# cemlyn007/ale-libtorch-ppo

Measured on AMD Instinct MI355X. Metric: env steps/sec (whole node), Breakout 84x84x4, higher is better.
Workload: dtype bf16; 1 GPU; Breakout-shaped synthetic, 128 envs/GPU x T=128, A=4, H=512, 4 epochs x 4 minibatches of 4096 (configs[1], v0.yaml update shape); envs_per_gpu=128, horizon=128, epochs=4, minibatches=4, parallelism=dp1, frames=raw u8 [E,2,210,160] pairs resident in HBM, rollout_planes=fp32, update_graph=False, dp_schedule_forced=False

## Files before the change

ale-libtorch-ppo_amd/csrc/api_core.hip:

```cpp
#include "api_internal.hpp"

using namespace aleppo;

namespace aleppo {

static thread_local std::string g_err;
int set_err(Ctx *c, int code, const std::string &msg) {
  if (c)
    c->err = msg;
  g_err = msg;
  return code;
}

static thread_local const Tuning *g_tuning = nullptr;
Tuning tuning_from_env() {
  auto flag = [](const char *name, bool dflt) {
    const char *e = std::getenv(name);
    return e ? std::atoi(e) != 0 : dflt;
  };
  Tuning t;
  t.patch_conv = !flag("ALEPPO_GENERIC_CONV", false);
  t.fc_pipe = flag("ALEPPO_FC_PIPE", true);
  t.fused_fwd = flag("ALEPPO_FWD_FUSED", true);
  if (const char *e = std::getenv("ALEPPO_BWD_FUSED"))
// ... 313 lines not shown
  CK(dalloc(&c->mask_counts, 4096 * 4, c->stream));
  CK(dalloc(&c->P, PT * 4, c->stream));
  CK(dalloc(&c->G, PT * 4, c->stream));
  CK(dalloc(&c->M1, PT * 4, c->stream));
  CK(dalloc(&c->M2, PT * 4, c->stream));
  if (c->prec == ALEPPO_BF16)
    CK(dalloc(reinterpret_cast<char **>(&c->Pc), PT * 2, c->stream));
  else
    c->Pc = c->P;
  CK(dalloc(reinterpret_cast<char **>(&c->W2d), (size_t)4 * 32 * 256 * ts, c->stream));
  CK(dalloc(reinterpret_cast<char **>(&c->W3d), (size_t)64 * 576 * ts, c->stream));
  CK(dalloc(reinterpret_cast<char **>(&c->WfcT), (size_t)FC_IN * H * ts, c->stream));
  const size_t mb = (size_t)c->maxB;
  CK(dalloc(reinterpret_cast<char **>(&c->a1), mb * A1_PIX * A1_C * ts, c->stream));
  CK(dalloc(reinterpret_cast<char **>(&c->a2), mb * A2_PIX * A2_C * ts, c->stream));
  CK(dalloc(reinterpret_cast<char **>(&c->a3), mb * FC_IN * ts, c->stream));
  CK(dalloc(reinterpret_cast<char **>(&c->dz1), mb * A1_PIX * A1_C * ts, c->stream));
  CK(dalloc(reinterpret_cast<char **>(&c->dz2), mb * A2_PIX * A2_C * ts, c->stream));
  CK(dalloc(reinterpret_cast<char **>(&c->dz3), mb * FC_IN * ts, c->stream));
  CK(dalloc(&c->h, (size_t)FC_FWD_MAX_PARTS * mb * H * 4, c->stream));
  CK(dalloc(&c->hpart, (size_t)FC_SPLITS * E * H * 4, c->stream));
  CK(dalloc(reinterpret_cast<char **>(&c->dh), mb * H * ts, c->stream));
  CK(dalloc(&c->logits_b, mb * A * 4, c->stream));
  CK(dalloc(&c->values_b, mb * 4, c->stream));
  c->slab_off[0] = 0;
  const size_t sl[10] = {(size_t)MAXS_C1 * 32 * 256,       (size_t)MAXS_C1 * 32, (size_t)MAXS_C2 * 64 * 512,
                         (size_t)MAXS_C2 * 64,              (size_t)MAXS_C3 * 64 * 576, (size_t)MAXS_C3 * 64,
                         (size_t)MAXS_FC * H * FC_IN,       (size_t)MAXS_HEAD * H, (size_t)MAXS_HEAD * (A + 1) * H,
                         (size_t)MAXS_HEAD * (A + 1)};
  for (int i = 0; i < 10; ++i)
    c->slab_off[i + 1] = c->slab_off[i] + align64(sl[i]);
  c->slab_floats = c->slab_off[10];
  CK(dalloc(&c->slab, c->slab_floats * 4, c->stream));
  CK(dalloc(&c->sumsq_part, 1024 * 4, c->stream));
  CK(dalloc(&c->adv_stats, 64, c->stream));
  CK(dalloc(&c->hyper_blk, HYPER_BLOCK * 4, c->stream));
  CK(hipHostMalloc(reinterpret_cast<void **>(&c->h_hyper_blk), HYPER_BLOCK * 4, hipHostMallocDefault));
  CK(hipStreamSynchronize(c->stream));
#undef CK
  *out = c;
  return ALEPPO_OK;
}

extern "C" void aleppo_destroy(aleppo_ctx *c) {
  if (!c)
    return;
  set_tuning(nullptr);
  (void)hipSetDevice(c->cfg.device_ordinal);
  if (c->h_go)
    __atomic_store_n(c->h_go, ~0ull, __ATOMIC_RELEASE);
  for (hipStream_t st : {c->wg_stream, c->comm_stream, c->stream})
    if (st)
      hipStreamSynchronize(st);
  if (c->graph_exec)
    hipGraphExecDestroy(c->graph_exec);
  if (c->graph)
    hipGraphDestroy(c->graph);
  if (c->nccl_comm)
    ncclCommDestroy(static_cast<ncclComm_t>(c->nccl_comm));
  void *dev[] = {c->obs,   c->step_rec, c->values_tm, c->logits_tm, c->actions_tm, c->lut,     c->d_start,
                 c->d_frames, c->d_noise, c->d_err,  c->d_done, c->adv_n,     c->ret_n,      c->oldlp_n, c->act_n,
                 c->mask_n, c->mask_counts, c->P,    c->G,         c->M1,      c->M2,
                 c->W2d,   c->W3d,      c->WfcT,      c->a1,        c->a2,         c->a3,      c->dz1,
                 c->dz2,   c->dz3,      c->h,         c->hpart,     c->dh,        c->logits_b,   c->values_b, c->slab,
                 c->sumsq_part, c->metric_ps, c->metric_red, c->grad_norms, c->adv_stats, c->stage_u8, c->stage_obs,
                 c->adam_sched, c->rb_tmp[0], c->rb_tmp[1], c->order, c->act_p, c->oldlp_p, c->adv_p,
                 c->ret_p,  c->mask_p,   c->mask_counts_ep, c->shuf_keys, c->val_n, c->val_p, c->advn_part,
// ... 319 lines not shown
```

ale-libtorch-ppo_amd/csrc/api_train.hip:

```cpp
#include "api_internal.hpp"

using namespace aleppo;

int aleppo::ensure_metric_storage(aleppo_ctx *c, int epochs, int M, long B) {
  const size_t need = (size_t)epochs * M * B;
  if (need > c->metric_cap) {
    retire(c, c->metric_ps);
    c->metric_ps = nullptr;
    HIPCHK(c, dalloc(&c->metric_ps, need * 7 * 4, c->stream));
    c->metric_cap = need;
  }
  const size_t nm = (size_t)epochs * M;
  if (nm > c->metric_red_cap) {
    retire(c, c->metric_red);
    retire(c, c->grad_norms);
    retire(c, c->adam_sched);
    retire(c, c->advn_part);
    retire(c, c->advn_stats);
    retire_host(c, c->h_metric_red);
    retire_host(c, c->h_adam_sched);
    retire_host(c, c->h_advn_stats);
    c->metric_red = c->grad_norms = c->h_metric_red = c->adam_sched = c->h_adam_sched = nullptr;
    c->advn_part = nullptr;
    c->advn_stats = c->h_advn_stats = nullptr;
// ... 50 lines not shown
    HIPCHK(c, hipHostMalloc(reinterpret_cast<void **>(&c->h_kl_beta), 16, hipHostMallocDefault));
  }
  if (c->kl_cap < c->metric_cap) {
    retire(c, c->kl_ps);
    c->kl_ps = nullptr;
    c->kl_cap = 0;
    c->last_kl = false;
    HIPCHK(c, dalloc(&c->kl_ps, c->metric_cap * 4, c->stream));
    c->kl_cap = c->metric_cap;
  }
  return ALEPPO_OK;
}

int aleppo::ensure_val_storage(aleppo_ctx *c) {
  if (!c->val_n)
    HIPCHK(c, dalloc(&c->val_n, (size_t)c->N * c->rsz, c->stream));
  return ALEPPO_OK;
}

static uint64_t splitmix64(uint64_t x) {
  uint64_t z = x + 0x9E3779B97F4A7C15ull;
  z = (z ^ (z >> 30)) * 0xBF58476D1CE4E5B9ull;
  z = (z ^ (z >> 27)) * 0x94D049BB133111EBull;
  return z ^ (z >> 31);
}
static int feistel_half_width(long N) {
  int w = 0;
  while ((1L << w) < N)
    ++w;
  w = std::max(w, 2);
  return (w + 1) / 2;
}

static bool fuse_tail_env() {
  static const bool v = [] {
    const char *e = getenv("ALEPPO_FUSE_TAIL_REDUCE");
    return !e || atoi(e) != 0;
  }();
  return v;
}
static bool bwd_streams_env() {
  static const bool v = [] {
    const char *e = std::getenv("ALEPPO_BWD_STREAMS");
    return !(e && std::atoi(e) == 1);
  }();
  return v;
}

static inline size_t record_index(bool per_epoch, size_t period, size_t i) { return per_epoch ? i : i % period; }

struct Planes {
  const int *act;
  void *oldlp, *adv, *ret, *vold;
  const uint8_t *mask;
  const int32_t *order;
  float *counts;
  int ncounts;
  size_t epoch_stride;
  long B;
  int M;
  size_t offset(int ep, int mb) const { return (size_t)ep * epoch_stride + (size_t)mb * B; }
  size_t record(int ep, int mb) const { return record_index(order != nullptr, (size_t)M, (size_t)ep * M + mb); }
  const int32_t *idx(int ep) const { return order ? order + (size_t)ep * epoch_stride : nullptr; }
};

struct UpdatePlan {
  int epochs, M, nm;
  long N, B;
  bool shuffle, vclip, val_transpose, advn, klpen, dp, two, bwd_fused, fuse_tail;
  hipStream_t s, sw;
  ncclComm_t comm;
  Hyper hp;
  const float *hpd;
  int shuf_h, nblk_head, nblk_sq;
  size_t fs;
  float *sW1, *sB1, *sW2, *sB2, *sW3, *sB3, *sWfc, *sBfc, *sWh, *sBh;
  Planes pl;
};

static int plan_update(aleppo_ctx *c, int epochs, int M, UpdatePlan *plan) {
  UpdatePlan &p = *plan;
  if (epochs <= 0 || M <= 0)
    return set_err(c, ALEPPO_ERR_INVALID_ARGUMENT, "epochs and num_mini_batches must be positive");
  const long N = c->batch_n;
  if (N <= 0)
    return set_err(c, ALEPPO_ERR_RUNTIME, "no batch: call aleppo_finish_rollout or aleppo_set_batch first");
  c->pre_acted = -1;
  if (N % M != 0)
    return set_err(c, ALEPPO_ERR_RUNTIME, "Batch size must be divisible by num_mini_batches");
  const long B = N / M;
  if (B > c->maxB)
    return set_err(c, ALEPPO_ERR_INVALID_ARGUMENT, "minibatch larger than config.max_minibatch");
  if (M > 4096)
    return set_err(c, ALEPPO_ERR_INVALID_ARGUMENT, "num_mini_batches > 4096");
  if (c->world > 1 && !c->nccl_comm)
    return set_err(c, ALEPPO_ERR_RUNTIME, "world_size > 1 but aleppo_comm_init was not called");
  p.epochs = epochs;
  p.M = M;
  p.nm = epochs * M;
  p.N = N;
  p.B = B;
  p.vclip = c->value_clip;
  if (p.vclip && c->val_src == Ctx::VAL_NONE)
    return set_err(c, ALEPPO_ERR_RUNTIME,
                   "ALEPPO_OPT_VALUE_CLIP needs the batch's old values: call aleppo_set_batch_values after aleppo_set_batch");
  int rc = ensure_metric_storage(c, epochs, M, B);
  if (rc)
    return rc;
  p.shuffle = c->shuffle;
  p.advn = c->adv_norm_mb;
  p.klpen = c->kl_pen;
  if (p.klpen && (rc = ensure_kl_storage(c)))
    return rc;
  if (p.shuffle && (rc = ensure_shuffle_storage(c, epochs, N)))
    return rc;
  if (p.vclip && (rc = ensure_val_storage(c)))
    return rc;
  p.val_transpose = p.vclip && c->val_src == Ctx::VAL_ROLLOUT;
  p.comm = static_cast<ncclComm_t>(c->nccl_comm);
  p.dp = c->world > 1 || (c->nccl_comm && c->force_comm);
  if (!c->wg_stream)
    HIPCHK(c, hipStreamCreateWithFlags(&c->wg_stream, hipStreamNonBlocking));
  if (p.dp && !c->comm_stream)
    HIPCHK(c, hipStreamCreateWithFlags(&c->comm_stream, hipStreamNonBlocking));
  p.s = c->stream;
  p.hp = c->hyper;
  p.hpd = c->hyper_blk;
  p.shuf_h = feistel_half_width(N);

  p.sW1 = c->slab + c->slab_off[0], p.sB1 = c->slab + c->slab_off[1], p.sW2 = c->slab + c->slab_off[2];
  p.sB2 = c->slab + c->slab_off[3], p.sW3 = c->slab + c->slab_off[4], p.sB3 = c->slab + c->slab_off[5];
  p.sWfc = c->slab + c->slab_off[6], p.sBfc = c->slab + c->slab_off[7], p.sWh = c->slab + c->slab_off[8];
  p.sBh = c->slab + c->slab_off[9];
  p.fs = c->metric_cap;
  p.nblk_head = (int)std::min<long>(MAXS_HEAD, (B + 15) / 16);
  p.nblk_sq = (int)std::min<size_t>(800, (c->L.off[P_W1] + 4095) / 4096);

  p.two = bwd_streams_env() && !c->serial_update;
  p.bwd_fused = (c->tune.fused_bwd == 2 || (c->tune.fused_bwd == 1 && B >= 2048)) && c->prec == ALEPPO_BF16 &&
                use_patch_kernels() && !p.dp;
  p.sw = p.two ? c->wg_stream : p.s;
  p.fuse_tail = fuse_tail_env();

  Planes &pl = p.pl;
  pl.B = B;
  pl.M = M;
  if (p.shuffle) {
    pl.act = c->act_p, pl.oldlp = c->oldlp_p, pl.adv = c->adv_p, pl.ret = c->ret_p, pl.vold = c->val_p;
    pl.mask = c->mask_p, pl.order = c->order, pl.counts = c->mask_counts_ep;
    pl.ncounts = p.nm;
    pl.epoch_stride = (size_t)N;
  } else {
    pl.act = c->act_n, pl.oldlp = c->oldlp_n, pl.adv = c->adv_n, pl.ret = c->ret_n, pl.vold = c->val_n;
    pl.mask = c->mask_n, pl.order = nullptr, pl.counts = c->mask_counts;
    pl.ncounts = M;
    pl.epoch_stride = 0;
  }
  if (!p.vclip)
    pl.vold = nullptr;
  return ALEPPO_OK;
}

static int upload_call_scalars(aleppo_ctx *c, const UpdatePlan &p, double lr) {
  hipStream_t s = p.s;
  for (int i = 0; i < p.nm; ++i) {
    const double b1 = c->cfg.adam_beta1, b2 = c->cfg.adam_beta2, t = (double)(c->adam_step + i + 1);
    c->h_adam_sched[2 * i] = (float)(lr / (1.0 - std::pow(b1, t)));
    c->h_adam_sched[2 * i + 1] = (float)std::sqrt(1.0 - std::pow(b2, t));
  }
  HIPCHK(c, hipMemcpyAsync(c->adam_sched, c->h_adam_sched, (size_t)p.nm * 8, hipMemcpyHostToDevice, s));
  float *b = c->h_hyper_blk;
  std::memset(b, 0, HYPER_BLOCK * 4);
  b[HYPER_CLIP] = p.hp.clip;
  b[HYPER_VCLIP] = c->vclip_range_set ? c->value_clip_range : p.hp.clip;
  b[HYPER_CV] = p.hp.c_v;
// ... 52 lines not shown
  const size_t p0 = pl.offset(ep, mb), fs = p.fs;
  float *const mps = c->metric_ps + (size_t)mi * p.B;
  HeadTrainArgs ha{};
  ha.h = c->h;
  ha.Wh = Pf(c, P_WH);
  ha.bh = Pf(c, P_BH);
  ha.act = pl.act + p0;
  ha.oldlp = rp(c, pl.oldlp, p0 * A);
  ha.adv = rp(c, pl.adv, p0);
  ha.ret = rp(c, pl.ret, p0);
  ha.vold = pl.vold ? rp(c, pl.vold, p0) : nullptr;
  ha.mask = pl.mask + p0;
  ha.mask_count = pl.counts + pl.record(ep, mb);
  ha.dh = c->dh;
  ha.prec = c->prec;
  ha.ps_total = mps + 0 * fs, ha.ps_clipped = mps + 1 * fs, ha.ps_value = mps + 2 * fs, ha.ps_entropy = mps + 3 * fs;
  ha.ps_ratio = mps + 4 * fs, ha.ps_kl = mps + 5 * fs, ha.ps_cf = mps + 6 * fs;
  ha.slab_w = p.sWh;
  ha.slab_b = p.sBh;
  ha.nblk = p.nblk_head;
  ha.B = p.B;
  ha.H = c->H;
  ha.A = A;
  ha.hparts = hparts;
  ha.rt16 = c->rt16;
  ha.advs = p.advn ? c->advn_stats + pl.record(ep, mb) * 4 : nullptr;
  ha.klb = p.klpen ? c->kl_beta : nullptr;
  ha.ps_kle = p.klpen ? c->kl_ps + (size_t)mi * p.B : nullptr;
  launch_head_train(p.s, ha, p.hpd);
  prof_end(c, ALEPPO_K_HEAD);
}

struct SegList {
  ReduceSeg seg[10];
  int n = 0;
  void add(const ReduceSeg &r) { seg[n++] = r; }
  void add(const SegList &o) {
    for (int i = 0; i < o.n; ++i)
      seg[n++] = o.seg[i];
  }
};
static void reduce_beside(aleppo_ctx *c, const UpdatePlan &p, SegList &segs) {
  if (!p.two)
    return;
  prof_begin(c, ALEPPO_K_REDUCE, p.sw);
  launch_reduce_slabs(p.sw, segs.seg, segs.n, c->G);
  prof_end(c, ALEPPO_K_REDUCE, p.sw);
  segs.n = 0;
}

static int enqueue_conv_bwd_fused(aleppo_ctx *c, const UpdatePlan &p, const SampleMap &map, int S3,
                                  const SegList &late0, SegList &segs, int *S1) {
  const ParamLayout &L = c->L;
  segs.add(ReduceSeg{p.sW3, S3, 64 * 576, (long)L.off[P_W3]});
  segs.add(ReduceSeg{p.sB3, S3, 64, (long)L.off[P_B3]});
  segs.add(late0);
  reduce_beside(c, p, segs);
  prof_begin(c, ALEPPO_K_CONV_BWD);
  const int S2 = *S1 = patch_conv_bwd_fused(p.s, c->dz2, c->a1, c->obs, map, c->W2d, p.sW2, p.sB2, p.sW1, p.sB1, p.B);
  prof_end(c, ALEPPO_K_CONV_BWD);
  segs.add(ReduceSeg{p.sW2, S2, 64 * 512, (long)L.off[P_W2]});
  segs.add(ReduceSeg{p.sB2, S2, 64, (long)L.off[P_B2]});
  return ALEPPO_OK;
}
static int enqueue_conv_bwd_split(aleppo_ctx *c, const UpdatePlan &p, const SampleMap &map, int S3,
                                  const SegList &late0, SegList &segs, int *S1) {
  const ParamLayout &L = c->L;
  const int prec = c->prec;
  HIPCHK(c, fork_wgrad_stream(p, c->ev_dz2));
  prof_begin(c, ALEPPO_K_CONV2_DGRAD);
  conv2_dgrad(p.s, prec, c->dz2, c->W2d, c->a1, c->dz1, p.B);
  prof_end(c, ALEPPO_K_CONV2_DGRAD);
  prof_begin(c, ALEPPO_K_CONV2_WGRAD, p.sw);
  const int S2 = conv2_wgrad(p.sw, prec, c->dz2, c->a1, p.sW2, p.sB2, p.B);
  prof_end(c, ALEPPO_K_CONV2_WGRAD, p.sw);
  segs.add(ReduceSeg{p.sW3, S3, 64 * 576, (long)L.off[P_W3]});
  segs.add(ReduceSeg{p.sB3, S3, 64, (long)L.off[P_B3]});
  segs.add(ReduceSeg{p.sW2, S2, 64 * 512, (long)L.off[P_W2]});
  segs.add(ReduceSeg{p.sB2, S2, 64, (long)L.off[P_B2]});
  segs.add(late0);
  reduce_beside(c, p, segs);
  prof_begin(c, ALEPPO_K_CONV1_WGRAD);
  *S1 = conv1_wgrad(p.s, prec, c->dz1, c->obs, map, p.sW1, p.sB1, p.B);
  prof_end(c, ALEPPO_K_CONV1_WGRAD);
  return ALEPPO_OK;
}

static int enqueue_minibatch(aleppo_ctx *c, const UpdatePlan &p, int ep, int mb) {
  const int H = c->H, A = c->A, prec = c->prec, mi = ep * p.M + mb;
  const ParamLayout &L = c->L;
  const long B = p.B;
  hipStream_t s = p.s, sw = p.sw;
  SampleMap map = train_map(c, (long)mb * B);
  map.idx = p.pl.idx(ep);
  const int hparts = net_forward(c, c->obs, map, B, FC_FWD_MAX_PARTS);
  enqueue_head(c, p, ep, mb, hparts);
  HIPCHK(c, fork_wgrad_stream(p, c->ev_head));
  prof_begin(c, ALEPPO_K_FC_DGRAD);
  fc_dgrad(s, prec, c->dh, c->WfcT, c->a3, c->dz3, B, H);
  prof_end(c, ALEPPO_K_FC_DGRAD);
  prof_begin(c, ALEPPO_K_FC_WGRAD, sw);
  const bool fc_direct = fc_wgrad_slices(prec, B) == 1;
  const int Sfc = fc_wgrad(sw, prec, c->dh, c->a3, fc_direct ? c->G + L.off[P_WFC] : p.sWfc,
                           fc_direct ? c->G + L.off[P_BFC] : p.sBfc, B, H);
  prof_end(c, ALEPPO_K_FC_WGRAD, sw);
  SegList segs0;
  segs0.add(ReduceSeg{p.sWh, p.nblk_head, (long)(A + 1) * H, (long)L.off[P_WH]});
  segs0.add(ReduceSeg{p.sBh, p.nblk_head, (long)A + 1, (long)L.off[P_BH]});
  if (!fc_direct) {
    segs0.add(ReduceSeg{p.sWfc, Sfc, (long)H * FC_IN, (long)L.off[P_WFC]});
    segs0.add(ReduceSeg{p.sBfc, Sfc, (long)H, (long)L.off[P_BFC]});
  }
  if (p.dp) {
    HIPCHK(c, hipEventRecord(c->ev_bucket0, sw));
    HIPCHK(c, hipStreamWaitEvent(c->comm_stream, c->ev_bucket0, 0));
    prof_begin(c, ALEPPO_K_REDUCE, c->comm_stream);
    launch_reduce_slabs(c->comm_stream, segs0.seg, segs0.n, c->G);
    prof_end(c, ALEPPO_K_REDUCE, c->comm_stream);
    NCCLCHK(c, ncclAllReduce(c->G, c->G, L.bucket0_end, ncclFloat, ncclSum, p.comm, c->comm_stream));
    HIPCHK(c, hipEventRecord(c->ev_comm0, c->comm_stream));
    segs0.n = 0;
  }
  HIPCHK(c, fork_wgrad_stream(p, c->ev_dz3));
  prof_begin(c, ALEPPO_K_CONV3_DGRAD);
  conv3_dgrad(s, prec, c->dz3, c->W3d, c->a2, c->dz2, B);
  prof_end(c, ALEPPO_K_CONV3_DGRAD);
  prof_begin(c, ALEPPO_K_CONV3_WGRAD, sw);
  const int S3 = conv3_wgrad(sw, prec, c->dz3, c->a2, p.sW3, p.sB3, B);
  prof_end(c, ALEPPO_K_CONV3_WGRAD, sw);
  int S1 = 0;
  SegList segs;
  if (int rc = p.bwd_fused ? enqueue_conv_bwd_fused(c, p, map, S3, segs0, segs, &S1)
                           : enqueue_conv_bwd_split(c, p, map, S3, segs0, segs, &S1))
    return rc;
  if (p.two) {
    HIPCHK(c, hipEventRecord(c->ev_wg, sw));
    HIPCHK(c, hipStreamWaitEvent(s, c->ev_wg, 0));
  }
  ReduceSeg tail[2] = {{p.sW1, S1, 32 * 256, (long)L.off[P_W1]}, {p.sB1, S1, 32, (long)L.off[P_B1]}};
  if (p.dp || !p.fuse_tail) {
    segs.add(tail[0]);
    segs.add(tail[1]);
    tail[0].slab = tail[1].slab = nullptr;
  }
  if (segs.n) {
    prof_begin(c, ALEPPO_K_REDUCE);
    launch_reduce_slabs(s, segs.seg, segs.n, c->G);
    prof_end(c, ALEPPO_K_REDUCE);
  }
  if (p.dp) {
    HIPCHK(c, hipStreamWaitEvent(s, c->ev_comm0, 0));
    NCCLCHK(c, ncclAllReduce(c->G + L.bucket0_end, c->G + L.bucket0_end, L.total() - L.bucket0_end, ncclFloat, ncclSum,
                             p.comm, s));
  }
  prof_begin(c, ALEPPO_K_ADAM);
  const int nblk_norm = launch_sumsq(s, c->G, (long)L.off[P_W1], c->sumsq_part, p.nblk_sq, tail);
  launch_adam(s, c->P, c->G, nullptr, c->M1, c->M2, c->prec == ALEPPO_BF16 ? c->Pc : nullptr, c->WfcT, c->W3d, c->W2d, L,
              prec, c->sumsq_part, nblk_norm, p.hpd, c->adam_sched + 2 * mi, c->cfg.adam_beta1, c->cfg.adam_beta2,
              c->cfg.adam_eps, c->grad_norms + mi);
  prof_end(c, ALEPPO_K_ADAM);
  return ALEPPO_OK;
}

static int enqueue_epilogue(aleppo_ctx *c, const UpdatePlan &p) {
  const Planes &pl = p.pl;
  launch_metrics_reduce(p.s, c->metric_ps, p.fs, pl.mask, p.B, pl.ncounts, p.nm / pl.ncounts, c->metric_red,
                        p.klpen ? c->kl_ps : nullptr);
  if (p.dp)
    NCCLCHK(c, ncclAllReduce(c->metric_red, c->metric_red, (size_t)p.nm * METRIC_REC, ncclFloat, ncclSum, p.comm, p.s));
  return ALEPPO_OK;
}

static int enqueue_update(aleppo_ctx *c, const UpdatePlan &p) {
  if (int rc = enqueue_prologue(c, p))
    return rc;
  for (int ep = 0; ep < p.epochs; ++ep)
    for (int mb = 0; mb < p.M; ++mb)
      if (int rc = enqueue_minibatch(c, p, ep, mb))
        return rc;
  return enqueue_epilogue(c, p);
}

static Ctx::GraphKey graph_key(const UpdatePlan &p, const aleppo_ctx *c) {
  Ctx::GraphKey key;
  key.epochs = p.epochs;
  key.M = p.M;
  key.two = p.two ? 1 : 0;
  key.N = p.N;
  key.metric_ps = c->metric_ps;
// ... 169 lines not shown
```

ale-libtorch-ppo_amd/csrc/common.hpp:

```cpp
#pragma once
#include "../../include/aleppo.h"
#include <hip/hip_runtime.h>
#include <stdint.h>
#include <string>
#include <vector>

namespace aleppo {

constexpr int FRAME_PIX = 84 * 84;
constexpr int RAW_H = 210, RAW_W = 160;
constexpr int A1_PIX = 400, A1_C = 32;
constexpr int A2_PIX = 81, A2_C = 64;
constexpr int A3_PIX = 49, A3_C = 64;
constexpr int FC_IN = 3136;
constexpr int MAX_ACTIONS = 18;
constexpr int FC_SPLITS = 7;
constexpr int MAXS_C1 = 256, MAXS_C2 = 256, MAXS_C3 = 256, MAXS_FC = 8, MAXS_HEAD = 256;
constexpr int METRIC_REC = 9;

enum ParamId { P_WH = 0, P_BH, P_WFC, P_BFC, P_W3, P_B3, P_W2, P_B2, P_W1, P_B1, P_COUNT };
struct ParamLayout {
  size_t off[P_COUNT + 1];
  size_t size[P_COUNT];
  size_t bucket0_end;
// ... 263 lines not shown
void launch_bstat_reduce(hipStream_t s, const double *part, int nblk, double *sums, double *result);
void launch_bstat_finalise(hipStream_t s, const double *sums, double *result);
void launch_shuffle_gather(hipStream_t s, const uint32_t *rk, int h, long N, int epochs, int A, int32_t *order,
                           const int *act_n, const void *oldlp_n, const void *adv_n, const void *ret_n,
                           const void *val_n, const uint8_t *mask_n, int *act_p, void *oldlp_p, void *adv_p,
                           void *ret_p, void *val_p, uint8_t *mask_p, bool rt16);
struct HeadTrainArgs {
  const float *h, *Wh, *bh;
  const int *act;
  const void *oldlp, *adv, *ret, *vold;
  const uint8_t *mask;
  const float *mask_count;
  void *dh;
  int prec;
  float *ps_total, *ps_clipped, *ps_value, *ps_entropy, *ps_ratio, *ps_kl, *ps_cf;
  float *slab_w, *slab_b;
  int nblk;
  long B;
  int H, A;
  float *logits_out = nullptr, *values_out = nullptr;
  int hparts = 1;
  bool rt16 = false;
  const float *advs = nullptr, *klb = nullptr;
  float *ps_kle = nullptr;
};
void launch_head_train(hipStream_t s, const HeadTrainArgs &a, const float *hp);
struct ReduceSeg {
  const float *slab;
  int S;
  long n;
  long dst;
};
void launch_reduce_slabs(hipStream_t s, const ReduceSeg *segs, int nseg, float *G);
int launch_sumsq(hipStream_t s, float *G, long n_main, float *partials, int nblk_main, const ReduceSeg tail[2],
                 int which = 0);
void launch_adam(hipStream_t s, float *P, const float *G_in, float *G_out_scaled, float *M1, float *M2, void *Pc,
                 void *WfcT, void *W3d, void *W2d, const ParamLayout &L, int prec, const float *partials, int nblk,
                 const float *hpd,
                 const float *sched,
                 float beta1, float beta2, float eps, float *grad_norm_out);
void launch_pack_dgrad(hipStream_t s, const float *P, const ParamLayout &L, void *W2d, void *W3d, void *WfcT,
                       int prec);
void launch_cast_params(hipStream_t s, const float *P, void *Pc, long n);
void launch_metrics_reduce(hipStream_t s, const float *ps, size_t field_stride, const uint8_t *mask_n, long B, int M,
                           int epochs, float *out, const float *kle = nullptr);
void launch_obs_unpack(hipStream_t s, const uint32_t *obs, uint8_t *out, long nsamp, SampleMap map);
void launch_obs_pack(hipStream_t s, const uint8_t *in, uint32_t *obs, long nsamp, SampleMap map);
void launch_transpose_tm_pitched(hipStream_t s, const void *src_tm, size_t pitch, void *dst_em, int E, int T, int inner,
                                 int elem);
void launch_state_digest(hipStream_t s, const float *P, const float *M1, const float *M2, const ParamLayout &L,
                         int64_t step, const uint32_t *obs, int slots, int slot, int E, uint64_t counter,
                         const double *rs_blk, const double *rs_g, unsigned long long *out);
void launch_heads_fwd(hipStream_t s, const float *h, const float *Wh, const float *bh, float *logits, float *values,
                      long n, int H, int A);
void launch_logsoftmax_rows(hipStream_t s, const float *in, float *out, long rows, int A);
void launch_area_resize(hipStream_t s, const float *in, float *out, long n);
void launch_rgb_to_gray(hipStream_t s, const float *in, float *out, long n);

void conv1_fwd(hipStream_t s, int prec, const uint32_t *obs, SampleMap map, const void *W1, const float *b1, void *a1,
               long ns);
void conv2_fwd(hipStream_t s, int prec, const void *a1, const void *W2, const float *b2, void *a2, long ns);
void conv3_fwd(hipStream_t s, int prec, const void *a2, const void *W3, const float *b3, void *a3, long ns);
int fc_fwd(hipStream_t s, int prec, const void *a3, const void *Wfc, const float *bfc, float *h, long ns, int H,
           int max_parts = 1);
constexpr int FC_FWD_MAX_PARTS = 4;
void fc_fwd_splitk(hipStream_t s, int prec, const void *a3, const void *Wfc, float *hpart, long ns, int H);
void fc_dgrad(hipStream_t s, int prec, const void *dh, const void *WfcT, const void *a3, void *dz3, long ns, int H);
void conv3_dgrad(hipStream_t s, int prec, const void *dz3, const void *W3d, const void *a2, void *dz2, long ns);
// ... 32 lines not shown
```

ale-libtorch-ppo_amd/csrc/kernels.hip:

```cpp
#include "common.hpp"
#include "gemm.hpp"
#include "head_train.hpp"
#include <algorithm>
#include <cstdlib>

namespace aleppo {

__device__ __forceinline__ float block_sum_256(float v, float *s4) {
  v = wave_sum(v);
  const int lane = threadIdx.x & 63, wave = threadIdx.x >> 6;
  __syncthreads();
  if (lane == 0)
    s4[wave] = v;
  __syncthreads();
  return (s4[0] + s4[1]) + (s4[2] + s4[3]);
}

template <bool RAW>
__global__ __launch_bounds__(256) void ingest_kernel(const uint8_t *__restrict__ frames, const uint8_t *__restrict__ lut,
                                                      const uint8_t *__restrict__ start, StartBits sbits, uint32_t *obs,
                                                      int slots, int t_src, int t_dst) {
  const int e = blockIdx.y, tid = threadIdx.x;
  const int pix = blockIdx.x * 256 + tid;
  __shared__ uint8_t slut[256];
// ... 956 lines not shown
    ret_p[row + i] = ret_n[j];
    if (val_n)
      val_p[row + i] = val_n[j];
    mask_p[row + i] = mask_n[j];
  }
  __syncthreads();
  const long cnt = min(256L, N - i0);
  for (long t = threadIdx.x; t < cnt * A; t += 256) {
    const long s = t / A, a = t - s * A;
    oldlp_p[(row + i0 + s) * A + a] = oldlp_n[(long)sj[s] * A + a];
  }
}
void launch_shuffle_gather(hipStream_t s, const uint32_t *rk, int h, long N, int epochs, int A, int32_t *order,
                           const int *act_n, const void *oldlp_n, const void *adv_n, const void *ret_n,
                           const void *val_n, const uint8_t *mask_n, int *act_p, void *oldlp_p, void *adv_p,
                           void *ret_p, void *val_p, uint8_t *mask_p, bool rt16) {
  const dim3 g((unsigned)((N + 255) / 256), (unsigned)epochs);
  if (rt16)
    hipLaunchKernelGGL(shuffle_gather_kernel<f16>, g, dim3(256), 0, s, rk, h, N, A, order, act_n,
                       static_cast<const f16 *>(oldlp_n), static_cast<const f16 *>(adv_n),
                       static_cast<const f16 *>(ret_n), static_cast<const f16 *>(val_n), mask_n, act_p,
                       static_cast<f16 *>(oldlp_p), static_cast<f16 *>(adv_p), static_cast<f16 *>(ret_p),
                       static_cast<f16 *>(val_p), mask_p);
  else
    hipLaunchKernelGGL(shuffle_gather_kernel<float>, g, dim3(256), 0, s, rk, h, N, A, order, act_n,
                       static_cast<const float *>(oldlp_n), static_cast<const float *>(adv_n),
                       static_cast<const float *>(ret_n), static_cast<const float *>(val_n), mask_n, act_p,
                       static_cast<float *>(oldlp_p), static_cast<float *>(adv_p), static_cast<float *>(ret_p),
                       static_cast<float *>(val_p), mask_p);
}


struct ReduceArgs {
  ReduceSeg seg[12];
  int cprefix[13];
  int wide[12];
  int nseg;
};
__global__ __launch_bounds__(256) void reduce_slabs_kernel(ReduceArgs a, float *G) {
  __shared__ float part[4][64];
  int s = 0;
  while ((int)blockIdx.x >= a.cprefix[s + 1])
    ++s;
  const long n = a.seg[s].n;
  const int S = a.seg[s].S;
  if (a.wide[s]) {
    const long j = ((long)((int)blockIdx.x - a.cprefix[s]) * 256 + threadIdx.x) * 4;
    if (j >= n)
      return;
    const float *p = a.seg[s].slab + j;
    float4 acc[4];
#pragma unroll
    for (int q = 0; q < 4; ++q)
      acc[q] = make_float4(0.f, 0.f, 0.f, 0.f);
    int k = 0;
    for (; k + 4 <= S; k += 4) {
      float4 v[4];
#pragma unroll
      for (int q = 0; q < 4; ++q)
        v[q] = *reinterpret_cast<const float4 *>(p + (long)(k + q) * n);
#pragma unroll
      for (int q = 0; q < 4; ++q) {
        acc[q].x += v[q].x;
        acc[q].y += v[q].y;
        acc[q].z += v[q].z;
        acc[q].w += v[q].w;
      }
    }
#pragma unroll
// ... 15 lines not shown
  }
  const long j = (long)((int)blockIdx.x - a.cprefix[s]) * 64 + (threadIdx.x & 63);
  const int q = threadIdx.x >> 6;
  float acc = 0.f;
  if (j < n) {
    const float *p = a.seg[s].slab + j;
#pragma unroll 4
    for (int k = q; k < S; k += 4)
      acc += p[(long)k * n];
  }
  part[q][threadIdx.x & 63] = acc;
  __syncthreads();
  if (q == 0 && j < n)
    G[a.seg[s].dst + j] = (part[0][threadIdx.x] + part[1][threadIdx.x]) + (part[2][threadIdx.x] + part[3][threadIdx.x]);
}
void launch_reduce_slabs(hipStream_t s, const ReduceSeg *segs, int nseg, float *G) {
  static const long wide_min = [] {
    const char *e = getenv("ALEPPO_REDUCE_WIDE_MIN");
    return e ? atol(e) : 1L << 18;
  }();
  ReduceArgs a;
  a.nseg = nseg;
  a.cprefix[0] = 0;
  for (int i = 0; i < nseg; ++i) {
    a.seg[i] = segs[i];
    const bool aligned = segs[i].n % 4 == 0 && segs[i].dst % 4 == 0 && ((uintptr_t)segs[i].slab & 15) == 0 &&
                         ((uintptr_t)G & 15) == 0;
    a.wide[i] = aligned && segs[i].n >= wide_min;
    a.cprefix[i + 1] = a.cprefix[i] + (int)(a.wide[i] ? (segs[i].n + 1023) / 1024 : (segs[i].n + 63) / 64);
  }
  hipLaunchKernelGGL(reduce_slabs_kernel, dim3(a.cprefix[nseg]), dim3(256), 0, s, a, G);
}

struct SumsqTail {
  ReduceSeg seg[2];
  int chunks[2];
};
__global__ __launch_bounds__(256) void sumsq_kernel(float *__restrict__ G, long n, float *partials, int nmain,
                                                    SumsqTail tail, int boff) {
  __shared__ float s4[4];
  __shared__ float part[4][64];
  float s = 0.f;
  const int blk = (int)blockIdx.x + boff;
  if (blk < nmain) {
    const long per = (n + nmain - 1) / nmain;
    const long b = (long)blk * per, e = min(n, b + per);
    for (long i = b + threadIdx.x; i < e; i += 256)
      s += G[i] * G[i];
  } else {
    int c = blk - nmain, t = 0;
    if (c >= tail.chunks[0]) {
      c -= tail.chunks[0];
      t = 1;
    }
    const ReduceSeg sg = tail.seg[t];
    const int o = threadIdx.x & 63, q = threadIdx.x >> 6;
    const long j = (long)c * 64 + o;
    float g = 0.f;
    if (sg.slab) {
      float acc = 0.f;
      if (j < sg.n) {
        const float *p = sg.slab + j;
#pragma unroll 4
        for (int k = q; k < sg.S; k += 4)
          acc += p[(long)k * sg.n];
      }
      part[q][o] = acc;
      __syncthreads();
      if (q == 0 && j < sg.n) {
        g = (part[0][o] + part[1][o]) + (part[2][o] + part[3][o]);
        G[sg.dst + j] = g;
      }
    } else if (q == 0 && j < sg.n) {
      g = G[sg.dst + j];
    }
    s = g * g;
  }
  s = block_sum_256(s, s4);
  if (threadIdx.x == 0)
    partials[blk] = s;
}
int launch_sumsq(hipStream_t s, float *G, long n_main, float *partials, int nblk_main, const ReduceSeg tail[2],
                 int which) {
  SumsqTail t;
  for (int i = 0; i < 2; ++i) {
    t.seg[i] = tail[i];
    t.chunks[i] = (int)((tail[i].n + 63) / 64);
  }
  const int ntail = t.chunks[0] + t.chunks[1], nblk = nblk_main + ntail;
  const int first = which == 2 ? nblk_main : 0, count = which == 1 ? nblk_main : nblk - first;
  hipLaunchKernelGGL(sumsq_kernel, dim3(count), dim3(256), 0, s, G, n_main, partials, nblk_main, t, first);
  return nblk;
}

struct long4_ranges {
  long begin[4], len[4];
};
struct AdamScalars {
  float coef, step_size, bc2_sqrt, beta1, beta2, omb1, omb2, eps;
};
__device__ __forceinline__ float adam_element(long i, float *P, const float *__restrict__ G, float *Gs, float *M1,
                                              float *M2, const AdamScalars &a) {
  const float g = G[i] * a.coef;
  const float m = M1[i] * a.beta1 + a.omb1 * g;
  const float v = M2[i] * a.beta2 + a.omb2 * (g * g);
  const float denom = sqrtf(v) / a.bc2_sqrt + a.eps;
  const float p = P[i] - a.step_size * (m / denom);
  M1[i] = m;
  M2[i] = v;
  P[i] = p;
  if (Gs)
    Gs[i] = g;
  return p;
}
struct AdamTiles {
  long off[3];
  int first[4];
  int H;
};
template <class T>
__global__ __launch_bounds__(256) void adam_kernel(float *P, const float *__restrict__ G, float *Gs, float *M1, float *M2,
                                                    T *Pc, T *WfcT, T *W3d, T *W2d, AdamTiles tl, long n_flat,
                                                    long4_ranges fr, const float *__restrict__ partials, int nblk,
                                                    const float *__restrict__ hpd, const float *__restrict__ sched,
                                                    float beta1, float beta2, float eps, float *grad_norm_out) {
  const float max_norm = hpd[HYPER_MAX_NORM];
  __shared__ float s4[4];
  __shared__ float tile[64][65];
  float s = 0.f;
  for (int i = threadIdx.x; i < nblk; i += 256)
    s += partials[i];
  s = block_sum_256(s, s4);
  const float norm = sqrtf(s);
  float coef = max_norm / (norm + 1e-6f);
  coef = fminf(coef, 1.0f);
  if (blockIdx.x == 0 && threadIdx.x == 0 && grad_norm_out)
    *grad_norm_out = norm;
  const AdamScalars a{coef, sched[0], sched[1], beta1, beta2, 1.0f - beta1, 1.0f - beta2, eps};
  const int ntile = tl.first[3];
  if ((int)blockIdx.x < ntile) {
    const int t = blockIdx.x;
    long src;
    int rs, rows, cols;
    T *dst;
    int ds;
    if (t < tl.first[1]) {
      const int ob = t / 49, jb = t - ob * 49;
      rs = FC_IN;
      rows = min(64, tl.H - ob * 64);
      cols = 64;
      src = tl.off[0] + (long)ob * 64 * FC_IN + jb * 64;
      dst = WfcT + (long)jb * 64 * tl.H + ob * 64;
      ds = tl.H;
    } else if (t < tl.first[2]) {
      const int tap = t - tl.first[1];
      rs = 576;
      rows = 64;
      cols = 64;
      src = tl.off[1] + tap * 64;
      dst = W3d + tap * 64;
      ds = 576;
    } else {
      const int k = t - tl.first[2], kh = k >> 2, kw = k & 3;
      const int cls = (kh & 1) * 2 + (kw & 1), ab = (kh >> 1) * 2 + (kw >> 1);
// ... 451 lines not shown
```

Baseline: 1.505 million env-steps/s.

## Replace sumsq with per-parameter norm pass that can fuse slab reductions

Replaces the grad-norm sumsq kernel, which read a flat range and fused only the conv1 tail, with a segmented norm pass over every parameter tensor in a fixed order. An env-selected level lets the per-block slab reductions for conv1, conv2/3 or all layers be done inside the norm pass instead of a separate reduce kernel. The fc weight uses wide float4 blocks. Adam's partial summation is vectorised. The default level 1 only routes conv1 as before, so the main change is the new segmented norm kernel layout. It also adds a partial-count capacity check.

```diff
diff --git a/ale-libtorch-ppo_amd/csrc/api_core.hip b/ale-libtorch-ppo_amd/csrc/api_core.hip
--- a/ale-libtorch-ppo_amd/csrc/api_core.hip
+++ b/ale-libtorch-ppo_amd/csrc/api_core.hip
@@ -369,7 +369,11 @@
     c->slab_off[i + 1] = c->slab_off[i] + align64(sl[i]);
   c->slab_floats = c->slab_off[10];
   CK(dalloc(&c->slab, c->slab_floats * 4, c->stream));
-  CK(dalloc(&c->sumsq_part, 1024 * 4, c->stream));
+  if (norm_pass_blocks(c->L) > NORM_PART_MAX) {
+    aleppo_destroy(c);
+    return set_err(nullptr, ALEPPO_ERR_RUNTIME, "norm pass: more partials than NORM_PART_MAX");
+  }
+  CK(dalloc(&c->sumsq_part, NORM_PART_MAX * 4, c->stream));
   CK(dalloc(&c->adv_stats, 64, c->stream));
   CK(dalloc(&c->hyper_blk, HYPER_BLOCK * 4, c->stream));
   CK(hipHostMalloc(reinterpret_cast<void **>(&c->h_hyper_blk), HYPER_BLOCK * 4, hipHostMallocDefault));
diff --git a/ale-libtorch-ppo_amd/csrc/api_train.hip b/ale-libtorch-ppo_amd/csrc/api_train.hip
--- a/ale-libtorch-ppo_amd/csrc/api_train.hip
+++ b/ale-libtorch-ppo_amd/csrc/api_train.hip
@@ -106,10 +106,11 @@
   return (w + 1) / 2;
 }
 
-static bool fuse_tail_env() {
-  static const bool v = [] {
+constexpr int FUSE_TAIL_DEFAULT = 1;
+static int fuse_tail_env() {
+  static const int v = [] {
     const char *e = getenv("ALEPPO_FUSE_TAIL_REDUCE");
-    return !e || atoi(e) != 0;
+    return e ? std::min(3, std::max(0, atoi(e))) : FUSE_TAIL_DEFAULT;
   }();
   return v;
 }
@@ -141,12 +142,13 @@
 struct UpdatePlan {
   int epochs, M, nm;
   long N, B;
-  bool shuffle, vclip, val_transpose, advn, klpen, dp, two, bwd_fused, fuse_tail;
+  bool shuffle, vclip, val_transpose, advn, klpen, dp, two, bwd_fused;
+  int fuse_tail;
   hipStream_t s, sw;
   ncclComm_t comm;
   Hyper hp;
   const float *hpd;
-  int shuf_h, nblk_head, nblk_sq;
+  int shuf_h, nblk_head;
   size_t fs;
   float *sW1, *sB1, *sW2, *sB2, *sW3, *sB3, *sWfc, *sBfc, *sWh, *sBh;
   Planes pl;
@@ -208,13 +210,12 @@
   p.sBh = c->slab + c->slab_off[9];
   p.fs = c->metric_cap;
   p.nblk_head = (int)std::min<long>(MAXS_HEAD, (B + 15) / 16);
-  p.nblk_sq = (int)std::min<size_t>(800, (c->L.off[P_W1] + 4095) / 4096);
 
   p.two = bwd_streams_env() && !c->serial_update;
   p.bwd_fused = (c->tune.fused_bwd == 2 || (c->tune.fused_bwd == 1 && B >= 2048)) && c->prec == ALEPPO_BF16 &&
                 use_patch_kernels() && !p.dp;
   p.sw = p.two ? c->wg_stream : p.s;
-  p.fuse_tail = fuse_tail_env();
+  p.fuse_tail = p.dp ? 0 : fuse_tail_env();
 
   Planes &pl = p.pl;
   pl.B = B;
@@ -333,7 +334,7 @@
 }
 
 struct SegList {
-  ReduceSeg seg[10];
+  ReduceSeg seg[P_COUNT];
   int n = 0;
   void add(const ReduceSeg &r) { seg[n++] = r; }
   void add(const SegList &o) {
@@ -341,8 +342,18 @@
       seg[n++] = o.seg[i];
   }
 };
+static void route_slabs(const UpdatePlan &p, const ParamLayout &L, ParamId id, const float *slab, int S, SegList &segs,
+                        NormSlabs &pass) {
+  const int from = id >= P_W1 ? 1 : id >= P_W2 ? 2 : 3;
+  if (p.fuse_tail >= from) {
+    pass.slab[id] = slab;
+    pass.S[id] = S;
+  } else {
+    segs.add(ReduceSeg{slab, S, (long)L.size[id], (long)L.off[id]});
+  }
+}
 static void reduce_beside(aleppo_ctx *c, const UpdatePlan &p, SegList &segs) {
-  if (!p.two)
+  if (!p.two || !segs.n)
     return;
   prof_begin(c, ALEPPO_K_REDUCE, p.sw);
   launch_reduce_slabs(p.sw, segs.seg, segs.n, c->G);
@@ -351,21 +362,21 @@
 }
 
 static int enqueue_conv_bwd_fused(aleppo_ctx *c, const UpdatePlan &p, const SampleMap &map, int S3,
-                                  const SegList &late0, SegList &segs, int *S1) {
+                                  const SegList &late0, SegList &segs, NormSlabs &pass, int *S1) {
   const ParamLayout &L = c->L;
-  segs.add(ReduceSeg{p.sW3, S3, 64 * 576, (long)L.off[P_W3]});
-  segs.add(ReduceSeg{p.sB3, S3, 64, (long)L.off[P_B3]});
+  route_slabs(p, L, P_W3, p.sW3, S3, segs, pass);
+  route_slabs(p, L, P_B3, p.sB3, S3, segs, pass);
   segs.add(late0);
   reduce_beside(c, p, segs);
   prof_begin(c, ALEPPO_K_CONV_BWD);
   const int S2 = *S1 = patch_conv_bwd_fused(p.s, c->dz2, c->a1, c->obs, map, c->W2d, p.sW2, p.sB2, p.sW1, p.sB1, p.B);
   prof_end(c, ALEPPO_K_CONV_BWD);
-  segs.add(ReduceSeg{p.sW2, S2, 64 * 512, (long)L.off[P_W2]});
-  segs.add(ReduceSeg{p.sB2, S2, 64, (long)L.off[P_B2]});
+  route_slabs(p, L, P_W2, p.sW2, S2, segs, pass);
+  route_slabs(p, L, P_B2, p.sB2, S2, segs, pass);
   return ALEPPO_OK;
 }
 static int enqueue_conv_bwd_split(aleppo_ctx *c, const UpdatePlan &p, const SampleMap &map, int S3,
-                                  const SegList &late0, SegList &segs, int *S1) {
+                                  const SegList &late0, SegList &segs, NormSlabs &pass, int *S1) {
   const ParamLayout &L = c->L;
   const int prec = c->prec;
   HIPCHK(c, fork_wgrad_stream(p, c->ev_dz2));
@@ -375,10 +386,10 @@
   prof_begin(c, ALEPPO_K_CONV2_WGRAD, p.sw);
   const int S2 = conv2_wgrad(p.sw, prec, c->dz2, c->a1, p.sW2, p.sB2, p.B);
   prof_end(c, ALEPPO_K_CONV2_WGRAD, p.sw);
-  segs.add(ReduceSeg{p.sW3, S3, 64 * 576, (long)L.off[P_W3]});
-  segs.add(ReduceSeg{p.sB3, S3, 64, (long)L.off[P_B3]});
-  segs.add(ReduceSeg{p.sW2, S2, 64 * 512, (long)L.off[P_W2]});
-  segs.add(ReduceSeg{p.sB2, S2, 64, (long)L.off[P_B2]});
+  route_slabs(p, L, P_W3, p.sW3, S3, segs, pass);
+  route_slabs(p, L, P_B3, p.sB3, S3, segs, pass);
+  route_slabs(p, L, P_W2, p.sW2, S2, segs, pass);
+  route_slabs(p, L, P_B2, p.sB2, S2, segs, pass);
   segs.add(late0);
   reduce_beside(c, p, segs);
   prof_begin(c, ALEPPO_K_CONV1_WGRAD);
@@ -388,7 +399,7 @@
 }
 
 static int enqueue_minibatch(aleppo_ctx *c, const UpdatePlan &p, int ep, int mb) {
-  const int H = c->H, A = c->A, prec = c->prec, mi = ep * p.M + mb;
+  const int H = c->H, prec = c->prec, mi = ep * p.M + mb;
   const ParamLayout &L = c->L;
   const long B = p.B;
   hipStream_t s = p.s, sw = p.sw;
@@ -406,11 +417,12 @@
                            fc_direct ? c->G + L.off[P_BFC] : p.sBfc, B, H);
   prof_end(c, ALEPPO_K_FC_WGRAD, sw);
   SegList segs0;
-  segs0.add(ReduceSeg{p.sWh, p.nblk_head, (long)(A + 1) * H, (long)L.off[P_WH]});
-  segs0.add(ReduceSeg{p.sBh, p.nblk_head, (long)A + 1, (long)L.off[P_BH]});
+  NormSlabs pass;
+  route_slabs(p, L, P_WH, p.sWh, p.nblk_head, segs0, pass);
+  route_slabs(p, L, P_BH, p.sBh, p.nblk_head, segs0, pass);
   if (!fc_direct) {
-    segs0.add(ReduceSeg{p.sWfc, Sfc, (long)H * FC_IN, (long)L.off[P_WFC]});
-    segs0.add(ReduceSeg{p.sBfc, Sfc, (long)H, (long)L.off[P_BFC]});
+    route_slabs(p, L, P_WFC, p.sWfc, Sfc, segs0, pass);
+    route_slabs(p, L, P_BFC, p.sBfc, Sfc, segs0, pass);
   }
   if (p.dp) {
     HIPCHK(c, hipEventRecord(c->ev_bucket0, sw));
@@ -431,19 +443,15 @@
   prof_end(c, ALEPPO_K_CONV3_WGRAD, sw);
   int S1 = 0;
   SegList segs;
-  if (int rc = p.bwd_fused ? enqueue_conv_bwd_fused(c, p, map, S3, segs0, segs, &S1)
-                           : enqueue_conv_bwd_split(c, p, map, S3, segs0, segs, &S1))
+  if (int rc = p.bwd_fused ? enqueue_conv_bwd_fused(c, p, map, S3, segs0, segs, pass, &S1)
+                           : enqueue_conv_bwd_split(c, p, map, S3, segs0, segs, pass, &S1))
     return rc;
   if (p.two) {
     HIPCHK(c, hipEventRecord(c->ev_wg, sw));
     HIPCHK(c, hipStreamWaitEvent(s, c->ev_wg, 0));
   }
-  ReduceSeg tail[2] = {{p.sW1, S1, 32 * 256, (long)L.off[P_W1]}, {p.sB1, S1, 32, (long)L.off[P_B1]}};
-  if (p.dp || !p.fuse_tail) {
-    segs.add(tail[0]);
-    segs.add(tail[1]);
-    tail[0].slab = tail[1].slab = nullptr;
-  }
+  route_slabs(p, L, P_W1, p.sW1, S1, segs, pass);
+  route_slabs(p, L, P_B1, p.sB1, S1, segs, pass);
   if (segs.n) {
     prof_begin(c, ALEPPO_K_REDUCE);
     launch_reduce_slabs(s, segs.seg, segs.n, c->G);
@@ -455,7 +463,9 @@
                              p.comm, s));
   }
   prof_begin(c, ALEPPO_K_ADAM);
-  const int nblk_norm = launch_sumsq(s, c->G, (long)L.off[P_W1], c->sumsq_part, p.nblk_sq, tail);
+  const int nblk_norm = launch_norm_pass(s, L, pass, c->G, c->sumsq_part);
+  if (nblk_norm < 0)
+    return set_err(c, ALEPPO_ERR_RUNTIME, "norm pass: the fc weight gradient is not 16-byte aligned");
   launch_adam(s, c->P, c->G, nullptr, c->M1, c->M2, c->prec == ALEPPO_BF16 ? c->Pc : nullptr, c->WfcT, c->W3d, c->W2d, L,
               prec, c->sumsq_part, nblk_norm, p.hpd, c->adam_sched + 2 * mi, c->cfg.adam_beta1, c->cfg.adam_beta2,
               c->cfg.adam_eps, c->grad_norms + mi);
diff --git a/ale-libtorch-ppo_amd/csrc/common.hpp b/ale-libtorch-ppo_amd/csrc/common.hpp
--- a/ale-libtorch-ppo_amd/csrc/common.hpp
+++ b/ale-libtorch-ppo_amd/csrc/common.hpp
@@ -319,8 +319,13 @@
   long dst;
 };
 void launch_reduce_slabs(hipStream_t s, const ReduceSeg *segs, int nseg, float *G);
-int launch_sumsq(hipStream_t s, float *G, long n_main, float *partials, int nblk_main, const ReduceSeg tail[2],
-                 int which = 0);
+struct NormSlabs {
+  const float *slab[P_COUNT] = {};
+  int S[P_COUNT] = {};
+};
+constexpr int NORM_PART_MAX = 2048;
+int norm_pass_blocks(const ParamLayout &L);
+int launch_norm_pass(hipStream_t s, const ParamLayout &L, const NormSlabs &sl, float *G, float *partials);
 void launch_adam(hipStream_t s, float *P, const float *G_in, float *G_out_scaled, float *M1, float *M2, void *Pc,
                  void *WfcT, void *W3d, void *W2d, const ParamLayout &L, int prec, const float *partials, int nblk,
                  const float *hpd,
diff --git a/ale-libtorch-ppo_amd/csrc/kernels.hip b/ale-libtorch-ppo_amd/csrc/kernels.hip
--- a/ale-libtorch-ppo_amd/csrc/kernels.hip
+++ b/ale-libtorch-ppo_amd/csrc/kernels.hip
@@ -1012,9 +1012,9 @@
 
 
 struct ReduceArgs {
-  ReduceSeg seg[12];
-  int cprefix[13];
-  int wide[12];
+  ReduceSeg seg[P_COUNT];
+  int cprefix[P_COUNT + 1];
+  int wide[P_COUNT];
   int nseg;
 };
 __global__ __launch_bounds__(256) void reduce_slabs_kernel(ReduceArgs a, float *G) {
@@ -1096,28 +1096,85 @@
   hipLaunchKernelGGL(reduce_slabs_kernel, dim3(a.cprefix[nseg]), dim3(256), 0, s, a, G);
 }
 
-struct SumsqTail {
-  ReduceSeg seg[2];
-  int chunks[2];
+constexpr int NORM_WIDE = 4096;
+constexpr int NORM_ORDER[P_COUNT] = {P_W1, P_W2, P_W3, P_WH, P_B1, P_B2, P_B3, P_BH, P_BFC, P_WFC};
+struct NormPassArgs {
+  ReduceSeg seg[P_COUNT];
+  int cprefix[P_COUNT + 1];
 };
-__global__ __launch_bounds__(256) void sumsq_kernel(float *__restrict__ G, long n, float *partials, int nmain,
-                                                    SumsqTail tail, int boff) {
+int norm_pass_blocks(const ParamLayout &L) {
+  long nb = 0;
+  for (int t = 0; t < P_COUNT; ++t)
+    nb += ((long)L.size[t] + (t == P_WFC ? NORM_WIDE : 64) - 1) / (t == P_WFC ? NORM_WIDE : 64);
+  return (int)nb;
+}
+__global__ __launch_bounds__(256) void norm_pass_kernel(NormPassArgs a, float *__restrict__ G, float *partials) {
   __shared__ float s4[4];
   __shared__ float part[4][64];
+  int t = 0;
+  while ((int)blockIdx.x >= a.cprefix[t + 1])
+    ++t;
+  const ReduceSeg sg = a.seg[t];
+  const int c = (int)blockIdx.x - a.cprefix[t];
   float s = 0.f;
-  const int blk = (int)blockIdx.x + boff;
-  if (blk < nmain) {
-    const long per = (n + nmain - 1) / nmain;
-    const long b = (long)blk * per, e = min(n, b + per);
-    for (long i = b + threadIdx.x; i < e; i += 256)
-      s += G[i] * G[i];
+  if (t == P_COUNT - 1) {
+    float4 ru[NORM_WIDE / 1024];
+#pragma unroll
+    for (int u = 0; u < NORM_WIDE / 1024; ++u) {
+      const long j = (long)c * NORM_WIDE + u * 1024 + threadIdx.x * 4;
+      float4 r = make_float4(0.f, 0.f, 0.f, 0.f);
+      if (j < sg.n) {
+        if (sg.slab) {
+          const float *p = sg.slab + j;
+          const long n = sg.n;
+          const int S = sg.S;
+          float4 acc[4];
+#pragma unroll
+          for (int q = 0; q < 4; ++q)
+            acc[q] = make_float4(0.f, 0.f, 0.f, 0.f);
+          int k = 0;
+          for (; k + 4 <= S; k += 4) {
+            float4 v[4];
+#pragma unroll
+            for (int q = 0; q < 4; ++q)
+              v[q] = *reinterpret_cast<const float4 *>(p + (long)(k + q) * n);
+#pragma unroll
+            for (int q = 0; q < 4; ++q) {
+              acc[q].x += v[q].x;
+              acc[q].y += v[q].y;
+              acc[q].z += v[q].z;
+              acc[q].w += v[q].w;
+            }
+          }
+#pragma unroll
+          for (int q = 0; q < 3; ++q)
+            if (k + q < S) {
+              const float4 v = *reinterpret_cast<const float4 *>(p + (long)(k + q) * n);
+              acc[q].x += v.x;
+              acc[q].y += v.y;
+              acc[q].z += v.z;
+              acc[q].w += v.w;
+            }
+          r.x = (acc[0].x + acc[1].x) + (acc[2].x + acc[3].x);
+          r.y = (acc[0].y + acc[1].y) + (acc[2].y + acc[3].y);
+          r.z = (acc[0].z + acc[1].z) + (acc[2].z + acc[3].z);
+          r.w = (acc[0].w + acc[1].w) + (acc[2].w + acc[3].w);
+          *reinterpret_cast<float4 *>(G + sg.dst + j) = r;
+        } else {
+          r = *reinterpret_cast<const float4 *>(G + sg.dst + j);
+        }
+      }
+      ru[u] = r;
+    }
+    float su[NORM_WIDE / 1024];
+#pragma unroll
+    for (int u = 0; u < NORM_WIDE / 1024; ++u) {
+      const float4 r = ru[u];
+      su[u] = __fmaf_rn(r.w, r.w, __fmaf_rn(r.z, r.z, __fmaf_rn(r.y, r.y, __fmul_rn(r.x, r.x))));
+    }
+    static_assert(NORM_WIDE == 4096, "the fold below takes four columns");
+    s = __fadd_rn(__fadd_rn(su[0], su[1]), __fadd_rn(su[2], su[3]));
   } else {
-    int c = blk - nmain, t = 0;
-    if (c >= tail.chunks[0]) {
-      c -= tail.chunks[0];
-      t = 1;
-    }
-    const ReduceSeg sg = tail.seg[t];
     const int o = threadIdx.x & 63, q = threadIdx.x >> 6;
     const long j = (long)c * 64 + o;
     float g = 0.f;
@@ -1138,23 +1195,26 @@
     } else if (q == 0 && j < sg.n) {
       g = G[sg.dst + j];
     }
-    s = g * g;
+    s = __fmul_rn(g, g);
   }
   s = block_sum_256(s, s4);
   if (threadIdx.x == 0)
-    partials[blk] = s;
-}
-int launch_sumsq(hipStream_t s, float *G, long n_main, float *partials, int nblk_main, const ReduceSeg tail[2],
-                 int which) {
-  SumsqTail t;
-  for (int i = 0; i < 2; ++i) {
-    t.seg[i] = tail[i];
-    t.chunks[i] = (int)((tail[i].n + 63) / 64);
-  }
-  const int ntail = t.chunks[0] + t.chunks[1], nblk = nblk_main + ntail;
-  const int first = which == 2 ? nblk_main : 0, count = which == 1 ? nblk_main : nblk - first;
-  hipLaunchKernelGGL(sumsq_kernel, dim3(count), dim3(256), 0, s, G, n_main, partials, nblk_main, t, first);
-  return nblk;
+    partials[blockIdx.x] = s;
+}
+int launch_norm_pass(hipStream_t s, const ParamLayout &L, const NormSlabs &sl, float *G, float *partials) {
+  NormPassArgs a;
+  a.cprefix[0] = 0;
+  static_assert(NORM_ORDER[P_COUNT - 1] == P_WFC, "the kernel takes the last segment for the fc weight");
+  for (int k = 0; k < P_COUNT; ++k) {
+    const int t = NORM_ORDER[k];
+    a.seg[k] = ReduceSeg{sl.slab[t], sl.S[t], (long)L.size[t], (long)L.off[t]};
+    const int per = t == P_WFC ? NORM_WIDE : 64;
+    a.cprefix[k + 1] = a.cprefix[k] + (int)((L.size[t] + per - 1) / per);
+  }
+  if (L.size[P_WFC] % 4 || L.off[P_WFC] % 4 || ((uintptr_t)sl.slab[P_WFC] & 15) || ((uintptr_t)G & 15))
+    return -1;
+  hipLaunchKernelGGL(norm_pass_kernel, dim3(a.cprefix[P_COUNT]), dim3(256), 0, s, a, G, partials);
+  return a.cprefix[P_COUNT];
 }
 
 struct long4_ranges {
@@ -1192,8 +1252,13 @@
   __shared__ float s4[4];
   __shared__ float tile[64][65];
   float s = 0.f;
-  for (int i = threadIdx.x; i < nblk; i += 256)
-    s += partials[i];
+  const int n4 = nblk & ~3;
+  for (int i = threadIdx.x * 4; i < n4; i += 1024) {
+    const float4 v = *reinterpret_cast<const float4 *>(partials + i);
+    s += (v.x + v.y) + (v.z + v.w);
+  }
+  if ((int)threadIdx.x < nblk - n4)
+    s += partials[n4 + threadIdx.x];
   s = block_sum_256(s, s4);
   const float norm = sqrtf(s);
   float coef = max_norm / (norm + 1e-6f);
```

Measured after the change: 1.516 million env-steps/s, median of 5. About the same (+0.7%).
